# blackccpie/another_raytracer

Measured on AMD Instinct MI355X. Metric: Msamples/sec (primary+secondary rays) at 1920x1080x1024spp; 1/2/4/8 GPU, higher is better.
Workload: dtype f64

## Files before the change

another_raytracer_amd/csrc/device.h:

```cpp
#pragma once
#include <hip/hip_runtime.h>

#include <cfloat>
#include <cstdint>
#include <type_traits>

#include "glibc_log.h"
#include "layout.h"
#include "sphere_uv.h"

namespace art {

struct V3 {
    double x, y, z;
};
__device__ __forceinline__ V3 mk(double a, double b, double c) { return V3{a, b, c}; }
__device__ __forceinline__ V3 operator+(V3 u, V3 v) { return {u.x + v.x, u.y + v.y, u.z + v.z}; }
__device__ __forceinline__ V3 operator-(V3 u, V3 v) { return {u.x - v.x, u.y - v.y, u.z - v.z}; }
__device__ __forceinline__ V3 operator-(V3 u) { return {-u.x, -u.y, -u.z}; }
__device__ __forceinline__ V3 operator*(V3 u, V3 v) { return {u.x * v.x, u.y * v.y, u.z * v.z}; }
__device__ __forceinline__ V3 operator*(double t, V3 v) { return {t * v.x, t * v.y, t * v.z}; }
__device__ __forceinline__ double sqrt_rn(double x) {
    if (!(x >= 0x1p-767 && x < __builtin_inf())) return sqrt(x);
    const double y = __builtin_amdgcn_rsq(x);
    double s = x * y, h = y * 0.5;
    const double r = fma(-h, s, 0.5);
    s = fma(s, r, s);
    h = fma(h, r, h);
    s = fma(fma(-s, s, x), h, s);
    return fma(fma(-s, s, x), h, s);
}
// ... 492 lines not shown
        *(__attribute__((address_space(3))) int32_t*)(size_t)(top + kRow) = v;
        top += keep ? kRow : 0u;
    }
    __device__ __forceinline__ int32_t peek() const { return *(__attribute__((address_space(3))) const int32_t*)(size_t)top; }
    __device__ __forceinline__ void pop_if(bool c) { top -= c ? kRow : 0u; }
    __device__ __forceinline__ uint32_t save() const { return top; }
    __device__ __forceinline__ void restore(uint32_t t) { top = t; }
};
template <bool L> using StackT = typename std::conditional<L, int16_t, int32_t>::type;
template <bool L, uint32_t F> using StackF = StackT<L || (F & F_CODE16) != 0>;
template <bool L>
__device__ __forceinline__ uint32_t stack_column(uint32_t t) {
    if (!L) return t;
    return (t & ~63u) | ((t & 31u) << 1) | ((t >> 5) & 1u);
}

__device__ __forceinline__ float f32_dir(double d) {
    const float f = static_cast<float>(d);
    return __builtin_copysignf(fmaxf(__builtin_fabsf(f), 0x1p-64f), f);
}
#ifndef ART_SUSPEND_LANES
#define ART_SUSPEND_LANES 24
#endif
struct TravResume {
    int32_t node, parked;
    uint32_t sp;
    int32_t lanes;
    bool fresh;
    bool allow;
    bool suspended;
};
template <uint32_t F, int B, bool L, int PL = 0, bool RES = false, int ANY = 0>
__device__ __forceinline__ bool traverse(const DevScene& S, const uint8_t* lds, int32_t root, const Ray& r, double tmin, double tmax,
                                         StackF<L, F>* stk, double& t, uint32_t& prim, uint32_t& face, uint32_t& mt, TravResume* rs = nullptr,
                                         int32_t hoisted = kNodeEmpty) {
    static_assert(!(L && (F & F_MEDIA)), "packed LDS keys need tmin > 0: no medium boundary tests in the LDS variant");
    static_assert(!RES || !L, "resumable traversal: HBM-scene variant only");
    static_assert(ANY == 0 || !RES, "any-hit walks are never suspended");
    constexpr bool kSort = ANY != 2;
    const float ox = static_cast<float>(r.o.x), oy = static_cast<float>(r.o.y), oz = static_cast<float>(r.o.z);
    const float ix = __builtin_amdgcn_rcpf(f32_dir(r.d.x)), iy = __builtin_amdgcn_rcpf(f32_dir(r.d.y)), iz = __builtin_amdgcn_rcpf(f32_dir(r.d.z));
    const float oix = ox * ix, oiy = oy * iy, oiz = oz * iz;
    constexpr uint32_t kLdsPlane = kLdsNodeCap * 16;
    static_assert(kLdsPlane % 256 == 0, "every node plane starts on bank 0");
    const uint32_t off_nx = kLdsOffNodes + (0u + (__float_as_uint(ix) >> 31)) * kLdsPlane;
    const uint32_t off_ny = kLdsOffNodes + (3u + (__float_as_uint(iy) >> 31)) * kLdsPlane;
    const uint32_t off_nz = kLdsOffNodes + (6u + (__float_as_uint(iz) >> 31)) * kLdsPlane;
    const float tminf = f_lo(tmin);
    float tmaxf = f_hi(tmax);
    constexpr bool kSphPre = !L && (F & F_SPHERE) != 0 && (F & F_TRI) == 0;
    constexpr bool kSphLazy = kSphPre && (F & (F_BOX | F_RECT | F_XFORM | F_MEDIA)) == 0;
    const double d_a = (L || kSphPre) ? len2(r.d) : 0.0;
    double d_inv_a = (L || (kSphPre && !kSphLazy)) ? 1.0 / d_a : 0.0;
    bool hit = false;
    constexpr bool PK = !L && (F & F_CODE16) != 0;
    constexpr uint32_t kLeafShift = (PK && (F & F_LEAF2) != 0) ? 1u : 0u;
    static_assert(!PK || (F & F_MEDIA_G) == 0, "packed keys need tmin > 0: no medium boundary traversals");
    LaneStack<B, L || PK> st(stk);
    constexpr bool kNfHoist = !L && PL == 2 && ((F & F_XFORM) == 0 || (F & (F_TRI | F_MEDIA_G)) == 0);
    [[maybe_unused]] const uint32_t nf_hx = (__float_as_uint(ix) >> 31) << 4, nf_hy = (__float_as_uint(iy) >> 31) << 4,
// ... 8 lines not shown
#define ART_DPUSH(q, keep) do { if (L) { dstk[dsp] = __uint_as_float(static_cast<uint32_t>(q) & 0xFFFF0000u); dsp += (keep) ? 1 : 0; } } while (0)
#define ART_DPOP(c) do { if (L && (c)) { cur_d = dsp > 0 ? dstk[dsp - 1] : 0.0f; dsp -= dsp > 0 ? 1 : 0; } } while (0)
#else
#define ART_DPUSH(q, keep) do { } while (0)
#define ART_DPOP(c) do { } while (0)
#endif
    int32_t parked = kNodeEmpty;
    [[maybe_unused]] bool skip_nodes = false;
    if (hoisted != kNodeEmpty && (!RES || rs->fresh)) {
        const int32_t h = L ? lds_leaf(leaf_first(hoisted), leaf_count(hoisted)) : PK ? make_leaf16(leaf_first(hoisted) >> kLeafShift, leaf_count(hoisted)) : hoisted;
        parked = h;
        skip_nodes = true;
    }
    if constexpr (RES) {
        if (!rs->fresh) {
            node = rs->node;
            parked = rs->parked;
            st.restore(rs->sp);
        }
    }
    [[maybe_unused]] bool progressed = false;
    ART_STAT_LANE(6);
    for (;;) {
        if constexpr (RES) {
            if (rs->allow && progressed && __popcll(__ballot(true)) < rs->lanes) {
                rs->node = node;
                rs->parked = parked;
                rs->sp = st.save();
                rs->fresh = false;
                rs->suspended = true;
                return hit;
            }
            progressed = true;
        }
        ART_STAT_WAVE(4);
        ART_STAT_LANE(5);
        while (node >= 0 && !skip_nodes) {
            ART_STAT_WAVE(0);
            ART_STAT_LANE(1);
#ifdef ART_STATS
            if (L && cur_d > tmaxf) ART_STAT_LANE(14);
#endif
            float4 lx, hx, ly, hy, lz, hz;
            int4 ch;
            if constexpr (L) {
                const uint32_t n16 = static_cast<uint32_t>(node);
                const uint32_t ax = n16 + off_nx, ay = n16 + off_ny, az = n16 + off_nz;
// ... 441 lines not shown
                ts.h.prim = kMediumHit;
                ts.h.obj = static_cast<uint32_t>(w);
                ts.h.mt = kMatUnknown;
            }
        } else {
            uint32_t prim = 0, face = 0, mt = kMatUnknown;
            if (hit_object<F, B, false, PL, true>(S, nullptr, oi, r, 0.001, ts.closest, stk, tt, prim, face, mt, &ts.tr)) {
                ts.closest = tt;
                ts.any = true;
                ts.h.prim = prim;
                ts.h.obj = static_cast<uint32_t>(w) | (face << 16);
                ts.h.mt = mt;
            }
            if (ts.tr.suspended) {
                ts.w = w;
                return false;
            }
            ts.tr.fresh = true;
        }
    }
    return true;
}

struct Surf {
    V3 p, n;
    double u, v;
    bool ff;
    uint32_t mat;
};
__device__ __forceinline__ void set_face_normal(Surf& s, const Ray& r, V3 outward) {
    s.ff = dot(r.d, outward) < 0.0;
    s.n = s.ff ? outward : -outward;
}
__device__ __forceinline__ void face_normal(const Ray& r, V3 outward, bool& ff, V3& n) {
    ff = dot(r.d, outward) < 0.0;
    n = ff ? outward : -outward;
}
template <bool UV = true>
__device__ __forceinline__ void rect_surface(V3& p, V3& n, bool& ff, double& su, double& sv, int axis, double a0, double a1, double b0, double b1, const Ray& r,
                                             double t, bool need_uv = true) {
    if (UV && need_uv) {
        const int ia = axis == 2 ? 1 : 0;
        const int ib = axis == 0 ? 1 : 2;
        const double x = comp(r.o, ia) + t * comp(r.d, ia);
        const double y = comp(r.o, ib) + t * comp(r.d, ib);
        su = (x - a0) / (a1 - a0);
// ... 246 lines not shown
```

another_raytracer_amd/csrc/k_paths.hip:

```cpp
#include "launch.h"
#include "path_pool.h"
#include "path_work.h"
#include "tile_lists.h"

namespace art {

struct __align__(16) PoolRay {
    double2 a, b, c;
    double2 d, e;
    uint64_t rng;
    uint32_t slot, depth;
};
static_assert(sizeof(PoolRay) == 96, "pool entries are six 16-B pieces");
struct PathPool {
    PoolRay* base;
    uint32_t count;
    uint32_t cur, end;
    bool exhausted;
    __device__ __forceinline__ void init(void* pool, uint32_t block, uint32_t nblocks, uint32_t waves_per_block, uint32_t w) {
        const uint32_t per_xcd = (nblocks + kXcds - 1) / kXcds;
        const uint32_t wave = ((block % kXcds) * per_xcd + block / kXcds) * waves_per_block + w;
        base = static_cast<PoolRay*>(pool) + static_cast<size_t>(wave) * kPoolCap;
        count = cur = end = 0;
        exhausted = false;
    }
    __device__ __forceinline__ bool batch(const PassGeom& sg, const CameraRec& sc, uint32_t* next_slot, uint32_t lane, PathState& st,
                                          uint32_t& q, uint32_t& tile) {
        if (cur == end) {
            const uint32_t chunk = sg.chunk;
            uint32_t nb = 0;
            if (lane == 0) nb = atomicAdd(next_slot, chunk);
            nb = __builtin_amdgcn_readfirstlane(nb);
            cur = nb;
            end = nb + chunk;
        }
        const uint32_t b = cur;
        cur += 64;
        q = b + lane;
        __asm__ volatile("" ::: "memory");
        if (b + 64u >= sg.P) exhausted = true;
        int lx, ly;
        uint32_t qi, j;
        slot_split(sg, q, qi, j);
        tile = __builtin_amdgcn_readfirstlane(qi >> 6);
        if (!(q < sg.P && slot_pixel(sg, qi, lx, ly))) return false;
        cam_ray(sg, sc, j, lx, ly, st.ray, st.rng);
        st.T = mk(1.0, 1.0, 1.0);
        return true;
    }
    __device__ __forceinline__ void push(uint64_t m, uint32_t rank, bool busy, const PathState& st, uint32_t q, int depth) {
        if (busy) {
            PoolRay& e = base[pool_push_pos(count, rank)];
            e.a = make_double2(st.ray.o.x, st.ray.o.y);
            e.b = make_double2(st.ray.o.z, st.ray.d.x);
            e.c = make_double2(st.ray.d.y, st.ray.d.z);
            e.d = make_double2(st.ray.tm, st.T.x);
            e.e = make_double2(st.T.y, st.T.z);
            e.rng = st.rng;
            e.slot = q;
            e.depth = static_cast<uint32_t>(depth);
        }
        count += static_cast<uint32_t>(__popcll(m));
        __asm__ volatile("" ::: "memory");
    }
    __device__ __forceinline__ void pop(uint32_t rank, PathState& st, uint32_t& q, int& depth) const {
        const PoolRay& e = base[pool_pop_pos(count, rank)];
        const double2 a = e.a, b = e.b, c = e.c, d = e.d, f = e.e;
        st.ray.o = mk(a.x, a.y, b.x);
        st.ray.d = mk(b.y, c.x, c.y);
        st.ray.tm = d.x;
        st.T = mk(d.y, f.x, f.y);
        st.rng = e.rng;
        q = e.slot;
        depth = static_cast<int>(e.depth);
    }
};
typedef uint32_t u32x8 __attribute__((ext_vector_type(8)));
__device__ __forceinline__ bool trace_tile_list(const uint8_t* lds, const Ray& r, u32x8 rec, double& t, HitOut& h) {
    const double d_a = len2(r.d), d_inv_a = 1.0 / d_a;
    uint64_t q0 = rec[0] | (static_cast<uint64_t>(rec[1]) << 32), q1 = rec[2] | (static_cast<uint64_t>(rec[3]) << 32);
    uint64_t q2 = rec[4] | (static_cast<uint64_t>(rec[5]) << 32), q3 = rec[6] | (static_cast<uint64_t>(rec[7]) << 32);
    const uint32_t n = static_cast<uint32_t>(q0) & 0xFFFFu;
    double closest = __builtin_inf();
    bool any = false;
    for (uint32_t k = 0; k < n; ++k) {
        q0 = (q0 >> 16) | (q1 << 48), q1 = (q1 >> 16) | (q2 << 48), q2 = (q2 >> 16) | (q3 << 48), q3 >>= 16;
// ... 24 lines not shown
    load_lds_image<B>(S0.lds_image, smem);
    if (threadIdx.x < static_cast<uint32_t>(kJumpEntries)) jt[threadIdx.x] = pcg_jump(3u * threadIdx.x);
    if (threadIdx.x == 0) {
        s_cam = cam;
        s_g = g;
        if (g.list_mode) {
            const uint32_t n = g.list[-1];
            s_g.nlist = n;
            s_g.P = n * g.k;
        }
    }
    DevScene S = S0;
    {
        uint8_t* wb = smem + paths_lds_head(g.stack);
        uint8_t* ob = wb + sizeof(int32_t) * kPathsWorldCap;
        if (threadIdx.x < static_cast<uint32_t>(S0.nworld)) reinterpret_cast<int32_t*>(wb)[threadIdx.x] = S0.world[threadIdx.x];
        if (threadIdx.x < S0.n_objs * (sizeof(ObjRec) / 16))
            reinterpret_cast<uint4*>(ob)[threadIdx.x] = reinterpret_cast<const uint4*>(S0.objs)[threadIdx.x];
        S.world = reinterpret_cast<const int32_t*>(wb);
        S.objs = reinterpret_cast<const ObjRec*>(ob);
    }
    __syncthreads();
    const uint32_t lane = __lane_id();
    const uint64_t below = (1ull << lane) - 1ull;
    const V3 bg = mk(S.bg[0], S.bg[1], S.bg[2]);
    bool busy = false;
    uint32_t q = 0;
    int depth = 0;
    PathState st;
    unsigned long long segs = 0;
#ifdef ART_STATS
    unsigned long long tm_load = 0, tm_trace = 0, tm_shade = 0, tm_app = 0, tm_fb = 0, tm_prev = __builtin_amdgcn_s_memtime();
#endif
    const bool lists = w.tiles != nullptr && g.list == nullptr;
    uint32_t tile = 0;
    PathPool pp;
    pp.init(w.pool, blockIdx.x, gridDim.x, B / 64, threadIdx.x / 64);
    for (;;) {
        const uint64_t m_busy = __ballot(busy);
        const uint32_t n_idle = 64u - static_cast<uint32_t>(__popcll(m_busy));
        const bool fb = pool_batch_due(pp.exhausted, pp.count, n_idle);
        bool act;
        if (fb) {
#ifdef ART_STATS
            if (lane == 0) atomicAdd(&g_art_stats[51], static_cast<unsigned long long>(__popcll(m_busy)));
#endif
            if (m_busy) pp.push(m_busy, static_cast<uint32_t>(__popcll(m_busy & below)), busy, st, q, depth);
            act = pp.batch(s_g, s_cam, next_slot, lane, st, q, tile);
            depth = 0;
        } else {
            const uint32_t npop = pool_pop_count(pp.count, n_idle);
            if (npop) {
                const uint32_t rank = static_cast<uint32_t>(__popcll(~m_busy & below));
                if (!busy && rank < npop) {
                    pp.pop(rank, st, q, depth);
                    busy = true;
                }
                pp.count -= npop;
            } else if (m_busy == 0) {
                ART_TICK(tm_load);
                break;
            }
            act = busy;
        }
        ART_TICK((fb ? tm_fb : tm_load));
        double t = 0.0;
        HitOut h{0, 0, kMatUnknown};
        bool hitw = false;
        if (act) {
            ++segs;
            u32x8 rec = {kTileOverflow, 0, 0, 0, 0, 0, 0, 0};
            if (fb && lists)
                rec = *(reinterpret_cast<const __attribute__((address_space(4))) u32x8*>(reinterpret_cast<uintptr_t>(w.tiles)) +
                        __builtin_amdgcn_readfirstlane(tile));
            if ((rec[0] & 0xFFFFu) != kTileOverflow) hitw = trace_tile_list(lds, st.ray, rec, t, h);
            else hitw = trace_world<kFeatSpheres, B, true>(S, lds, st.ray, stk, st.rng, t, h);
#if ART_LDS_LEAF_NOREF
            if (hitw) h.mt = reinterpret_cast<const uint32_t*>(lds + kLdsOffRef)[h.obj >> 16] >> kLdsRefMatShift;
#endif
        }
        __asm__ volatile("s_waitcnt vmcnt(0)" ::: "memory");
        ART_TICK((fb ? tm_fb : tm_trace));
        const bool need = act && hitw && (h.mt == MAT_LAMBERTIAN || h.mt == MAT_METAL) && depth + 1 < g.max_depth;
        const V3 ps = coop_unit_sphere(need, st.rng, jt);
        bool cont = false;
        if (act) {
            st.L = mk(0.0, 0.0, 0.0);
            if (hitw) {
                cont = shade_hit_lds(lds, h.obj >> 16, h.mt, t, depth + 1 >= g.max_depth, st, &ps);
            } else {
                st.L = st.L + st.T * bg;
            }
            if (!cont) store_res(w.res, q, st.L);
        }
        ART_TICK((fb ? tm_fb : tm_shade));
#ifdef ART_STATS
        if (fb) {
            const uint64_t m_act = __ballot(act);
            if (lane == 0) {
                atomicAdd(&g_art_stats[49], 1ull);
                atomicAdd(&g_art_stats[50], static_cast<unsigned long long>(__popcll(m_act)));
            }
        }
#endif
        if (fb || act) {
            busy = cont;
            ++depth;
        }
        ART_TICK((fb ? tm_fb : tm_app));
    }
    for (int off = 32; off > 0; off >>= 1) segs += __shfl_xor(segs, off);
    if (lane == 0) atomicAdd(w.segments, segs);
#ifdef ART_STATS
    if (lane == 0) {
        atomicAdd(&g_art_stats[8], tm_load);
        atomicAdd(&g_art_stats[9], tm_trace);
        atomicAdd(&g_art_stats[10], tm_shade);
        atomicAdd(&g_art_stats[11], tm_app);
        atomicAdd(&g_art_stats[48], tm_fb);
    }
#endif
}

void launch_paths(int num_cu, hipStream_t st, const DevScene& S, const PassGeom& g, const CameraRec& cam, const Work& w,
                  uint32_t* next_slot) {
    const size_t lds = paths_lds_bytes(g.stack);
    static const bool checked = static_lds_is_zero(reinterpret_cast<const void*>(k_paths));
    (void)checked;
    (void)blocks_per_cu(reinterpret_cast<const void*>(k_paths), kBlockL, lds);
    hipLaunchKernelGGL(k_paths, dim3(num_cu), dim3(kBlockL), lds, st, S, g, cam, w, next_slot);
}
size_t pool_bytes(int variant, int num_cu) {
    return variant == EXT_MEGA ? sizeof(PoolRay) * kPoolCap * kPoolWavesPerCu * static_cast<size_t>(num_cu) : 0;
}

}
```

another_raytracer_amd/csrc/options.cpp:

```cpp
#include "options.h"

#include <algorithm>
#include <atomic>
#include <cmath>
#include <cstdlib>
#include <cstring>
#include <limits>

namespace art {

namespace {

struct OptDef {
    const char* name;
    double def, lo, hi;
    bool integer;
};
constexpr double kInf = std::numeric_limits<double>::infinity();
const OptDef kDefs[static_cast<int>(Opt::kCount)] = {
    {"compile.world_merge", 2, 0, 2, true},
    {"compile.hoist", 1, 0, 1, true},
    {"bvh.collapse", 0, 0, 1, true},
    {"bvh.collapse_ci", 0.6, 0, 1e6, false},
    {"bvh.dp_binary_leaf", 1, 1, 16, true},
    {"bvh.sah_ci", 1.5, 0, 1e6, false},
    {"bvh.sah_leaf", 4, 1, 16, true},
    {"bvh.sbvh", 1.5, 0, 1e6, false},
    {"bvh.sbvh_alpha", 1e-5, 0, 1e6, false},
    {"render.codes16", 1, 0, 1, true},
    {"render.lds_nodes_max", 4294967295.0, 0, 4294967295.0, true},
    {"render.leaf2", 1, 0, 1, true},
    {"render.tex_bary", 1, 0, 1, true},
    {"denoise.lds_iterations", 2, 0, 2, true},
    {"query.any_sorted", 0, 0, 1, true},
    {"views.max_paths", 0, 0, 2147483648.0, true},
    {"render.tile_lists", 1, 0, 2, true},
    {"render.accum_overlap", 1, 0, 2, true},
    {"grad.texel_copies", 0, 0, 64, true},
    {"multi.timeout_ms", std::numeric_limits<double>::quiet_NaN(), 0, kInf, false},
    {"multi.rccl_blocking", 0, 0, 1, true},
    {"test.fault_workspace_bytes", 0, 0, 1.8e19, true},
    {"test.fault_gather_abort", 0, 0, 1, true},
    {"test.fault_rccl_group", 0, 0, 2, true},
};

std::atomic<double> g_val[static_cast<int>(Opt::kCount)];
std::atomic<bool> g_init{false};

void init_once() {
    if (g_init.load(std::memory_order_acquire)) return;
    static const bool done = [] {
        opt_reset_all();
        g_init.store(true, std::memory_order_release);
        return true;
    }();
    (void)done;
}

int find(const char* name) {
    if (!name) return -1;
    for (int i = 0; i < static_cast<int>(Opt::kCount); ++i)
        if (std::strcmp(kDefs[i].name, name) == 0) return i;
    return -1;
}

}

void opt_reset_all() {
    for (int i = 0; i < static_cast<int>(Opt::kCount); ++i) g_val[i].store(kDefs[i].def, std::memory_order_relaxed);
}

double opt(Opt o) {
    init_once();
    const double v = g_val[static_cast<int>(o)].load(std::memory_order_relaxed);
    if (o == Opt::MultiTimeoutMs && std::isnan(v)) {
        const char* s = std::getenv("ART_MULTI_TIMEOUT_MS");
        return (!s || !*s) ? 120000.0 : std::max(0.0, std::strtod(s, nullptr));
    }
    return v;
}

bool opt_set(const char* name, double value, const char** why) {
    init_once();
    const int i = find(name);
    if (i < 0) {
        *why = "unknown option";
        return false;
    }
    const OptDef& d = kDefs[i];
    if (!(value >= d.lo && value <= d.hi) || (d.integer && value != std::floor(value))) {
        *why = d.integer ? "value outside the option's integer range" : "value outside the option's range";
        return false;
// ... 15 lines not shown
```

another_raytracer_amd/csrc/options.h:

```cpp
#pragma once
#include <cstddef>

namespace art {

enum class Opt : int {
    WorldMerge,
    Hoist,
    BvhCollapse,
    CollapseCi,
    DpBinaryLeaf,
    SahCi,
    SahLeaf,
    Sbvh,
    SbvhAlpha,
    Codes16,
    LdsNodesMax,
    Leaf2,
    TexBary,
    DenoiseLdsIterations,
    QueryAnySorted,
    ViewsMaxPaths,
    TileLists,
    AccumOverlap,
    GradTexelCopies,
    MultiTimeoutMs,
    RcclBlocking,
    FaultWorkspaceBytes,
    FaultGatherAbort,
    FaultRcclGroup,
    kCount
};

double opt(Opt o);
bool opt_set(const char* name, double value, const char** why);
bool opt_get(const char* name, double* value);
void opt_reset_all();

}
```

another_raytracer_amd/csrc/path_work.h:

```cpp
#pragma once
#include <hip/hip_runtime.h>

#include <cstdint>

#include "device.h"
#include "pass_plan.h"

namespace art {

struct PathRec {
    double2 a, b, c, e;
    double2 f, g, h, i;
};
static_assert(sizeof(PathRec) == 128, "PathRec is two 64-B lines");
struct PathState {
    Ray ray;
    V3 T, L;
    uint64_t rng;
};
__device__ __forceinline__ void load_path(const PathRec* P, uint32_t q, PathState& s, bool full) {
    const PathRec& p = P[q];
    const double2 a = p.a, b = p.b, c = p.c, e = p.e;
    s.ray.o = mk(a.x, a.y, b.x);
    s.ray.d = mk(b.y, c.x, c.y);
    s.ray.tm = e.x;
// ... 50 lines not shown

struct FastDiv {
    uint32_t d, m, l;
    static FastDiv make(uint32_t d) {
        uint32_t l = 0;
        while (l < 32 && (1ull << l) < d) ++l;
        return FastDiv{d, static_cast<uint32_t>(((1ull << 32) * ((1ull << l) - d)) / d + 1), l};
    }
    __device__ __forceinline__ uint32_t div(uint32_t n) const { return (__umulhi(m, n) + n) >> l; }
};

struct PassGeom {
    int32_t W, H;
    int32_t rows;
    int32_t band_rows, band_count, band_index;
    uint32_t tiles_x, npix_pad;
    uint32_t k;
    uint32_t sample_base;
    uint32_t P;
    uint32_t cap;
    uint32_t live;
    uint32_t stack;
    int32_t max_depth;
    uint64_t seed;
    uint64_t seed_mix;
    FastDiv fd_npix, fd_tiles_x, fd_band_rows, fd_w;
    double inv_w1, inv_h1;
    const uint32_t* list;
    uint32_t nlist;
    uint32_t chunk;
    uint32_t lds_ring;
    uint32_t list_mode;
};
struct Work {
    PathRec* paths;
    HitRecD* hits;
    ResRec* res;
    uint32_t* active[2];
    uint32_t* mq;
    uint32_t* counters;
    unsigned long long* segments;
    double* acc;
    void* pool;
    const void* tiles;
};
__host__ __device__ __forceinline__ uint32_t* counter(const Work& w, int d, int kind, int s) {
    return w.counters + (static_cast<size_t>((d * kQueueKinds + kind) * kShards + s)) * kCounterStride;
}

__device__ __forceinline__ int global_row(const PassGeom& g, int ly) {
    const uint32_t b = g.fd_band_rows.div(static_cast<uint32_t>(ly));
    return static_cast<int>(b) * (g.band_rows * g.band_count) + g.band_index * g.band_rows + (ly - static_cast<int>(b) * g.band_rows);
}
__device__ __forceinline__ void slot_split(const PassGeom& g, uint32_t slot, uint32_t& qi, uint32_t& j) {
    const uint32_t a = g.fd_npix.div(slot), b = slot - a * g.npix_pad;
    qi = g.list_mode ? a : b;
// ... 271 lines not shown
```

another_raytracer_amd/csrc/renderer.hip:

```cpp
#include "renderer.h"

#include <algorithm>
#include <cstdio>
#include <cstdlib>
#include <cstring>
#include <vector>

#include "call_plan.h"
#include "launch.h"
#include "lds_image.h"
#include "options.h"
#include "pass_plan.h"
#include "refit.h"
#include "tile_lists.h"
#include "view_plan.h"
#include "workspace.h"

namespace art {

struct Renderer::Impl {
    int device = 0;
    int num_cu = 256;
    hipStream_t own_stream = nullptr;
    FlatScene flat;
// ... 118 lines not shown
        unsigned long long segments = 0;
        void fill(RenderStats* s, uint64_t primary, int passes, int samples_per_pass) const {
            if (s) *s = RenderStats{}, s->segments = segments, s->primary = primary, s->ms = ms, s->passes = passes, s->samples_per_pass = samples_per_pass;
        }
    };
    Done finish(const unsigned long long* d_segments = nullptr) {
        Done d;
        if (timed && d_segments) HIP_OK(hipMemcpyAsync(&d.segments, d_segments, sizeof d.segments, hipMemcpyDeviceToHost, st));
        if (wait) HIP_OK(hipStreamSynchronize(st));
        if (timed) HIP_OK(hipEventElapsedTime(&d.ms, ev[0], ev[1]));
        return d;
    }
};
static uint64_t slot_target(const Renderer::Impl& I, size_t slot_bytes) {
    size_t free_b = 0, total_b = 0;
    HIP_OK(hipMemGetInfo(&free_b, &total_b));
    return slot_target(free_b, I.ws.size(), slot_bytes);
}

size_t Renderer::scene_bytes() const { return impl_->s64.bytes; }
int Renderer::device() const { return impl_->device; }
const FlatScene& Renderer::flat() const { return impl_->flat; }

static PassGeom make_pass_geom(const RenderParams& p, int nrows, uint32_t stack) {
    PassGeom g{};
    g.W = p.width;
    g.H = p.height;
    g.rows = nrows;
    g.band_rows = p.band_rows;
    g.band_count = p.band_count;
    g.band_index = p.band_index;
    g.tiles_x = static_cast<uint32_t>((p.width + 7) / 8);
    const uint32_t tiles_y = static_cast<uint32_t>((nrows + 7) / 8);
    g.npix_pad = g.tiles_x * tiles_y * 64u;
    g.max_depth = p.max_depth;
    g.seed = p.seed;
    g.seed_mix = splitmix64(p.seed);
    g.fd_tiles_x = FastDiv::make(g.tiles_x);
    g.fd_band_rows = FastDiv::make(static_cast<uint32_t>(p.band_rows));
    g.fd_w = FastDiv::make(static_cast<uint32_t>(p.width));
    g.fd_npix = FastDiv::make(g.npix_pad);
    g.inv_w1 = 1.0 / static_cast<double>(p.width - 1);
    g.inv_h1 = 1.0 / static_cast<double>(p.height - 1);
    g.stack = stack;
    return g;
}
constexpr uint32_t kTileListsAutoSpp = 72;
static bool tile_lists_wanted(const DeviceScene& ds, int variant, uint32_t k) {
    const int mode = static_cast<int>(opt(Opt::TileLists));
    return variant == EXT_MEGA && ds.tile_reps > 0 && (mode == 2 || (mode == 1 && k >= kTileListsAutoSpp));
}
static size_t counter_words(int max_depth) { return static_cast<size_t>(std::max(max_depth + 1, 4)) * kQueueKinds * kShards * kCounterStride; }

struct ProfileMarks {
    std::vector<hipEvent_t> ev;
    size_t used = 0;
    ~ProfileMarks() { for (auto e : ev) if (e) (void)hipEventDestroy(e); }
    void reserve(size_t n) {
        while (ev.size() < n) {
            ev.push_back(nullptr);
            HIP_OK(hipEventCreate(&ev.back()));
        }
    }
    void mark(hipStream_t stream) {
        reserve(used + 1);
        HIP_OK(hipEventRecord(ev[used++], stream));
    }
// ... 82 lines not shown
    f.stream = f.call.st;
    for (int a = 0; a < 3; ++a) f.ds.view.bg[a] = p.background[a];
    f.nrows = band_local_rows(p.height, p.band_rows, p.band_count, p.band_index);
    stats.local_rows = f.nrows;
    if (f.nrows == 0) return false;
    f.g = make_pass_geom(p, f.nrows, stack_rows(f.ds.max_stack));
    f.variant = extend_variant(f.ds, p.flags);
    f.mega = f.variant == EXT_MEGA || f.variant == EXT_MEGA_G;
    const size_t slot_bytes = f.mega ? sizeof(ResRec) : sizeof(PathRec) + sizeof(HitRecD) + sizeof(ResRec) + 4u * (2u + kNumMatTypes) + 8u;
    const uint64_t target = slot_target(I, slot_bytes);
    if (f.g.npix_pad > kMaxPassSlots) throw std::runtime_error("image too large for one pass (more than 2^31 padded pixels)");
    const PassPlan plan = plan_passes(target, p.samples_per_pass, f.g.npix_pad, spp, spread);
    f.k = plan.k, f.npasses = plan.npasses;
    f.Pmax = f.k * f.g.npix_pad;
    f.g.cap = shard_cap(f.Pmax);
    f.local_pix = static_cast<size_t>(f.nrows) * p.width;
    f.counter_bytes = f.mega ? 4u * kCounterStride : 4ull * counter_words(p.max_depth);
    f.call.carve(I.ws, carve);
    if (p.flags & RT_PROFILE) {
        f.marks.reserve(static_cast<size_t>(profile_levels) * f.npasses * (f.variant == EXT_MEGA ? 4 : f.mega ? 2 : 3 * p.max_depth));
        f.mark = [&f]() { f.marks.mark(f.stream); };
    }
    f.call.begin();
    HIP_OK(hipMemsetAsync(f.w.segments, 0, sizeof(unsigned long long), f.stream));
    if (p.max_depth == 0) HIP_OK(hipMemsetAsync(f.w.res, 0, sizeof(ResRec) * f.Pmax, f.stream));
    return true;
}

static void run_pass(Frame& f, PassGeom g, int line = 0, bool clear = true, size_t res_first = 0) {
    Work w = f.w;
    w.res += res_first;
    if (clear) HIP_OK(hipMemsetAsync(f.w.counters, 0, f.counter_bytes, f.stream));
    if (!f.mega) {
        for (int d = 0; d < f.p.max_depth; ++d) bounce(f.ds, f.variant, f.I.num_cu, f.stream, g, f.cam, w, d, f.mark);
        f.launches += static_cast<uint64_t>(f.p.max_depth);
    } else if (f.p.max_depth > 0) {
        g.chunk = path_chunk(g.P, f.I.num_cu);
        if (f.mark) f.mark();
        if (f.variant == EXT_MEGA) {
            launch_paths(f.I.num_cu, f.stream, f.ds.view, g, f.cam, w, counter(w, line, 0, 0));
            f.kid = KernelId{kFeatSpheres, 0, 3};
        } else {
            f.kid = launch_paths_g(f.ds.features, f.ds.tex_basic, f.ds.tex_bary, f.ds.codes16, f.ds.leaf_shift, f.I.num_cu, f.stream, f.ds.view, g,
                                   f.cam, w, counter(w, line, 0, 0));
        }
        if (f.mark) f.mark();
        ++f.launches;
    }
    ++f.passes;
}

static PassGeom list_geom(PassGeom g, const uint32_t* list, uint32_t nlist, uint32_t k, uint32_t sample_base, uint32_t P) {
    g.list_mode = 1, g.list = list, g.nlist = nlist;
    g.k = g.npix_pad = k, g.fd_npix = FastDiv::make(k), g.sample_base = sample_base;
    g.P = g.live = P;
    return g;
}

static void end_frame(Frame& f, RenderStats& stats, uint8_t* out_rgb, double* out_acc, const std::function<void()>& more_copies = {}) {
#ifdef ART_STATS
    HIP_OK(hipGetLastError());
    dump_art_stats(f.stream);
#endif
    f.call.end();
    f.call.copy_out(out_rgb, f.drgb, 3 * f.local_pix);
    f.call.copy_out(out_acc, f.w.acc, sizeof(double) * 3 * f.local_pix);
    if (more_copies) more_copies();
    const Call::Done done = f.call.finish(f.w.segments);
    stats.ms = done.ms, stats.segments = done.segments, stats.passes = f.passes, stats.samples_per_pass = static_cast<int>(f.k);
    stats.extend_variant = f.variant, stats.kernel_features = f.kid.f, stats.kernel_textures = f.kid.tf, stats.kernel_lds_mode = f.kid.lm;
    if (f.p.flags & RT_PROFILE) {
        f.marks.sum(f.mega ? 2 : 3, stats.extend_ms, stats.shade_ms);
        stats.extend_launches = f.launches;
        stats.shade_launches = f.variant == EXT_GLOBAL || f.variant == EXT_LDS ? f.launches : 0;
    }
}

struct RenderBufs {
    int spp_t;
    uint8_t* out_rgb;
    double *out_acc, *qsum;
    int32_t* ad_work;
    uint32_t *ad_lists, *ad_count;
    uint8_t *ad_f0, *ad_f1, *ad_f2;
    int sqx;
    uint32_t nsq;
};

static int trace_samples(Frame& f, const RenderBufs& b, const uint32_t* list, uint32_t nlist) {
    const RenderParams& p = f.p;
    PassGeom g = f.g;
// ... 102 lines not shown
}

void Renderer::render(const CameraRec& cam, const RenderParams& p, uint8_t* out_rgb, double* out_acc, RenderStats& stats) {
    if (p.fp_mode != RT_FP64) throw std::runtime_error("fp_mode must be RT_FP64");
    upload();
    Impl& I = *impl_;
    Frame f{I, I.s64, cam, p};
    const bool images = (p.flags & RT_PARALLEL_IMAGES) != 0, adaptive = (p.flags & RT_ADAPTIVE) != 0;
    RenderBufs b{};
    b.spp_t = images ? 4 * (p.spp / 4) : p.spp, b.out_rgb = out_rgb, b.out_acc = out_acc;
#ifdef ART_TRACE
    trace_setup();
#endif
    TileRec* tile_tab = nullptr;
    if (!begin_frame(f, stats, b.spp_t, true, adaptive ? 4 : 1, [&](Carver& c) {
        const bool wf = !f.mega;
        f.w.paths = c.take<PathRec>(f.Pmax, wf);
        f.w.hits = c.take<HitRecD>(f.Pmax, wf);
        f.w.res = c.take<ResRec>(f.Pmax);
        f.w.active[0] = c.take<uint32_t>(static_cast<size_t>(kShards) * f.g.cap, wf);
        f.w.active[1] = c.take<uint32_t>(static_cast<size_t>(kShards) * f.g.cap, wf);
        f.w.mq = c.take<uint32_t>(static_cast<size_t>(kMatSegs) * f.g.cap, wf);
        f.w.counters = c.take<uint32_t>(counter_words(p.max_depth));
        f.w.segments = c.take<unsigned long long>(1);
        f.w.acc = c.take<double>(3 * f.local_pix);
        f.drgb = c.take<uint8_t>(3 * f.local_pix);
        double* qsum = c.take<double>(3 * f.local_pix, images);
        b.qsum = images ? qsum : nullptr;
        f.w.pool = c.take<char>(pool_bytes(f.variant, I.num_cu));
        tile_tab = c.take<TileRec>(f.g.npix_pad / 64u, !adaptive && tile_lists_wanted(f.ds, f.variant, f.k));
        b.ad_work = c.take<int32_t>(3 * f.local_pix, adaptive);
        b.ad_lists = c.take<uint32_t>(adaptive_list_words(static_cast<uint32_t>(f.local_pix / (kBig * kBig))), adaptive);
        b.ad_f0 = c.take<uint8_t>(21 * (f.local_pix / (kBig * kBig)), adaptive);
        b.ad_count = c.take<uint32_t>(1, adaptive);
    })) return;
    b.ad_f1 = b.ad_f0 + f.local_pix / (kBig * kBig), b.ad_f2 = b.ad_f1 + 4 * (f.local_pix / (kBig * kBig));
    b.sqx = p.width / kBig, b.nsq = static_cast<uint32_t>(b.sqx) * static_cast<uint32_t>(f.nrows / kBig);
    uint32_t ad_counts[4] = {0, 0, 0, 0};
    uint64_t primary = 0;
    if (!adaptive && p.max_depth > 0 && tile_lists_wanted(f.ds, f.variant, f.k)) {
        launch_tile_lists(f.stream, f.ds.view, f.g, cam, tile_tab);
        f.w.tiles = tile_tab;
    }
    if (!adaptive) primary = render_whole(f, b);
    else if (f.mega && f.k == static_cast<uint32_t>(b.spp_t) && !images && !p.on_pass) adaptive_device_counted(f, b, ad_counts);
    else primary = adaptive_host_counted(f, b);
    end_frame(f, stats, out_rgb, adaptive ? nullptr : out_acc);
// ... 279 lines not shown
    DeviceBuffer tmp;
    double* d_rays = nullptr;
    uint64_t* d_rng = nullptr;
    call.carve(tmp, [&](Carver& c) { d_rays = call.out(c, rays_out, 7 * ne), d_rng = call.out(c, rng_out, ne); }, 1);
    launch_camera_rays(call.st, g, cam, d_rays, d_rng);
    call.end();
    call.finish();
}

void Renderer::render_noise_target(const CameraRec& cam, const RenderParams& p, const NoiseParams& np, uint8_t* out_rgb, double* out_acc,
                                   int32_t* out_count, double* out_moments, RenderStats& stats, NoiseResult& result) {
    if (p.fp_mode != RT_FP64) throw std::runtime_error("fp_mode must be RT_FP64");
    upload();
    Impl& I = *impl_;
    Frame f{I, I.s64, cam, p};
    result = NoiseResult{};
    double* mom = nullptr;
    int32_t* count = nullptr;
    uint8_t* flag = nullptr;
    uint32_t *list_base = nullptr, *conv = nullptr;
    if (!begin_frame(f, stats, p.spp, false, 0, [&](Carver& c) {
        f.w.res = c.take<ResRec>(f.Pmax);
        f.w.counters = c.take<uint32_t>(kCounterStride);
        f.w.segments = c.take<unsigned long long>(1);
        f.w.acc = c.take<double>(3 * f.local_pix);
        mom = c.take<double>(2 * f.local_pix);
        count = c.take<int32_t>(f.local_pix);
        flag = c.take<uint8_t>(f.local_pix);
        f.drgb = c.take<uint8_t>(3 * f.local_pix);
        list_base = c.take<uint32_t>(nt_list_words(f.local_pix));
        conv = c.take<uint32_t>(1);
        f.w.pool = c.take<char>(pool_bytes(f.variant, I.num_cu));
    })) return;
    if (!f.mega) throw std::runtime_error("internal: noise-target rendering needs a persistent-path kernel");
    hipStream_t stream = f.stream;
    const Work& w = f.w;
    const size_t local_pix = f.local_pix;
    const uint32_t npix = static_cast<uint32_t>(local_pix), tile_pad = f.g.npix_pad;
    const double* res = reinterpret_cast<const double*>(w.res);
    uint32_t* lists[2] = {list_base + 64, list_base + nt_list_stride(local_pix) + 64};
    HIP_OK(hipMemsetAsync(w.acc, 0, sizeof(double) * 3 * local_pix, stream));
    HIP_OK(hipMemsetAsync(mom, 0, sizeof(double) * 2 * local_pix, stream));
    HIP_OK(hipMemsetAsync(flag, 0, local_pix, stream));
    HIP_OK(hipMemsetAsync(list_base, 0, 4 * nt_list_words(local_pix), stream));
    HIP_OK(hipMemsetAsync(conv, 0, 4, stream));
    const uint32_t min_spp = static_cast<uint32_t>(np.min_spp), cap_spp = static_cast<uint32_t>(p.spp), step = static_cast<uint32_t>(np.step_spp);
    PassGeom g = f.g;
// ... 281 lines not shown
```

Baseline: 23820.

## Suspend partial LDS BVH walks into the path pool when wave occupancy drops

Lets the persistent-path kernel's LDS-scene traversal suspend when fewer than a threshold of lanes are active. The partial walk (closest t, node, parked leaf, world index, short stack) is saved into a new per-wave PoolWalk area beside the pooled rays, so idle lanes can be refilled with fresh paths and suspended walks are resumed later. The aim is to cut SIMD divergence from long-tail traversals. In exchange it adds pool memory, per-iteration ballots, stack copy traffic and new bookkeeping for which pool slots hold walks. The hold threshold defaults to 8 lanes through a new option, and diagnostic counters for held and displaced paths are added.

```diff
diff --git a/another_raytracer_amd/csrc/device.h b/another_raytracer_amd/csrc/device.h
--- a/another_raytracer_amd/csrc/device.h
+++ b/another_raytracer_amd/csrc/device.h
@@ -7,6 +7,7 @@
 
 #include "glibc_log.h"
 #include "layout.h"
+#include "path_hold.h"
 #include "sphere_uv.h"
 
 namespace art {
@@ -545,6 +546,8 @@
 #ifndef ART_SUSPEND_LANES
 #define ART_SUSPEND_LANES 24
 #endif
+template <int B>
+__host__ __device__ constexpr uint32_t hold_stack_row(uint32_t depth) { return kLdsImageBytes + depth * 2u * B; }
 struct TravResume {
     int32_t node, parked;
     uint32_t sp;
@@ -558,7 +561,6 @@
                                          StackF<L, F>* stk, double& t, uint32_t& prim, uint32_t& face, uint32_t& mt, TravResume* rs = nullptr,
                                          int32_t hoisted = kNodeEmpty) {
     static_assert(!(L && (F & F_MEDIA)), "packed LDS keys need tmin > 0: no medium boundary tests in the LDS variant");
-    static_assert(!RES || !L, "resumable traversal: HBM-scene variant only");
     static_assert(ANY == 0 || !RES, "any-hit walks are never suspended");
     constexpr bool kSort = ANY != 2;
     const float ox = static_cast<float>(r.o.x), oy = static_cast<float>(r.o.y), oz = static_cast<float>(r.o.z);
@@ -613,7 +615,19 @@
     [[maybe_unused]] bool progressed = false;
     ART_STAT_LANE(6);
     for (;;) {
-        if constexpr (RES) {
+        if constexpr (RES && L) {
+            const bool more = (node != kNodeEmpty || parked != kNodeEmpty) &&
+                              static_cast<int32_t>(st.top) < static_cast<int32_t>(hold_stack_row<B>(kHoldStackCap + 1));
+            if (rs->allow && progressed && __popcll(__ballot(true)) < rs->lanes && more) {
+                rs->node = node;
+                rs->parked = parked;
+                rs->sp = st.save();
+                rs->fresh = false;
+                rs->suspended = true;
+                return hit;
+            }
+            progressed = true;
+        } else if constexpr (RES) {
             if (rs->allow && progressed && __popcll(__ballot(true)) < rs->lanes) {
                 rs->node = node;
                 rs->parked = parked;
@@ -1101,6 +1115,29 @@
     return true;
 }
 
+template <uint32_t F, int B>
+__device__ __forceinline__ bool trace_world_res_lds(const DevScene& S, const uint8_t* lds, const Ray& r, StackT<true>* stk, TraceState& ts) {
+    ts.tr.suspended = false;
+    for (int32_t w = ts.w; w < S.nworld; ++w) {
+        const int32_t oi = S.world[w];
+        double tt;
+        uint32_t prim = 0, face = 0, mt = kMatUnknown;
+        if (hit_object<F, B, true, 0, true>(S, lds, oi, r, 0.001, ts.closest, stk, tt, prim, face, mt, &ts.tr)) {
+            ts.closest = tt;
+            ts.any = true;
+            ts.h.prim = prim;
+            ts.h.obj = static_cast<uint32_t>(w) | (face << 16);
+            ts.h.mt = mt;
+        }
+        if (ts.tr.suspended) {
+            ts.w = w;
+            return false;
+        }
+        ts.tr.fresh = true;
+    }
+    return true;
+}
+
 struct Surf {
     V3 p, n;
     double u, v;
diff --git a/another_raytracer_amd/csrc/k_paths.hip b/another_raytracer_amd/csrc/k_paths.hip
--- a/another_raytracer_amd/csrc/k_paths.hip
+++ b/another_raytracer_amd/csrc/k_paths.hip
@@ -12,18 +12,34 @@
     uint32_t slot, depth;
 };
 static_assert(sizeof(PoolRay) == 96, "pool entries are six 16-B pieces");
+struct __align__(16) PoolWalk {
+    double t;
+    uint32_t np;
+    uint32_t misc;
+    uint32_t stk[kHoldStackCap / 2];
+};
+static_assert(sizeof(PoolWalk) == 64, "walk entries are four 16-B pieces");
+static_assert(kPathsWorldCap <= kWalkWorldCap, "walk_pack's world slots (path_hold.h)");
+constexpr unsigned long long kSegsDisplaced = 1ull << 40;
+constexpr size_t kPoolWaveBytes = (sizeof(PoolRay) + sizeof(PoolWalk)) * kPoolCap;
+__device__ __forceinline__ uint32_t lanes_below(uint64_t m) {
+    return __builtin_amdgcn_mbcnt_hi(static_cast<uint32_t>(m >> 32), __builtin_amdgcn_mbcnt_lo(static_cast<uint32_t>(m), 0u));
+}
 struct PathPool {
     PoolRay* base;
+    uint64_t held;
     uint32_t count;
     uint32_t cur, end;
     bool exhausted;
     __device__ __forceinline__ void init(void* pool, uint32_t block, uint32_t nblocks, uint32_t waves_per_block, uint32_t w) {
         const uint32_t per_xcd = (nblocks + kXcds - 1) / kXcds;
-        const uint32_t wave = ((block % kXcds) * per_xcd + block / kXcds) * waves_per_block + w;
-        base = static_cast<PoolRay*>(pool) + static_cast<size_t>(wave) * kPoolCap;
+        const uint32_t wave = ((block % kXcds) * per_xcd + block / kXcds) * waves_per_block + __builtin_amdgcn_readfirstlane(w);
+        base = reinterpret_cast<PoolRay*>(static_cast<uint8_t*>(pool) + static_cast<size_t>(wave) * kPoolWaveBytes);
+        held = 0;
         count = cur = end = 0;
         exhausted = false;
     }
+    __device__ __forceinline__ PoolWalk* walks() const { return reinterpret_cast<PoolWalk*>(base + kPoolCap); }
     __device__ __forceinline__ bool batch(const PassGeom& sg, const CameraRec& sc, uint32_t* next_slot, uint32_t lane, PathState& st,
                                           uint32_t& q, uint32_t& tile) {
         if (cur == end) {
@@ -48,7 +64,31 @@
         st.T = mk(1.0, 1.0, 1.0);
         return true;
     }
-    __device__ __forceinline__ void push(uint64_t m, uint32_t rank, bool busy, const PathState& st, uint32_t q, int depth) {
+    __device__ __forceinline__ void push(uint64_t m, uint64_t m_held, bool busy, bool walk, const PathState& st, uint32_t q,
+                                         int depth, double t, uint32_t np, uint32_t misc, const StackT<true>* stk) {
+        const uint32_t n_held = static_cast<uint32_t>(__popcll(m_held));
+        const uint32_t rank = hold_push_rank(walk, lanes_below(m_held), n_held, lanes_below(m & ~m_held));
+        if (m_held) {
+            if (walk) {
+                PoolWalk& x = walks()[pool_push_pos(count, rank)];
+                *reinterpret_cast<uint4*>(&x) = make_uint4(static_cast<uint32_t>(__double_as_longlong(t)),
+                                                           static_cast<uint32_t>(__double_as_longlong(t) >> 32), np, misc);
+                const uint32_t n = walk_entries(misc);
+                for (uint32_t k0 = 0; k0 < kHoldStackCap; k0 += 8) {
+                    if (k0 >= n) break;
+                    uint32_t v[4];
+#pragma unroll
+                    for (uint32_t c = 0; c < 4; ++c) {
+                        const uint32_t k = k0 + 2 * c;
+                        const uint32_t lo = k < n ? static_cast<uint16_t>(stk[k * kBlockL]) : 0u;
+                        const uint32_t hi = k + 1 < n ? static_cast<uint16_t>(stk[(k + 1) * kBlockL]) : 0u;
+                        v[c] = lo | (hi << 16);
+                    }
+                    *reinterpret_cast<uint4*>(&x.stk[k0 / 2]) = make_uint4(v[0], v[1], v[2], v[3]);
+                }
+            }
+            held = hold_mask_push(held, count, n_held);
+        }
         if (busy) {
             PoolRay& e = base[pool_push_pos(count, rank)];
             e.a = make_double2(st.ray.o.x, st.ray.o.y);
@@ -62,6 +102,25 @@
         }
         count += static_cast<uint32_t>(__popcll(m));
         __asm__ volatile("" ::: "memory");
+    }
+    __device__ __forceinline__ void pop_walk(uint32_t pos, double& t, uint32_t& np, uint32_t& misc, StackT<true>* stk) const {
+        const PoolWalk& x = walks()[pos];
+        const uint4 hd = *reinterpret_cast<const uint4*>(&x);
+        t = __longlong_as_double(static_cast<long long>(hd.x | (static_cast<uint64_t>(hd.y) << 32)));
+        np = hd.z;
+        misc = hd.w;
+        const uint32_t n = walk_entries(misc);
+        for (uint32_t k0 = 0; k0 < kHoldStackCap; k0 += 8) {
+            if (k0 >= n) break;
+            const uint4 s = *reinterpret_cast<const uint4*>(&x.stk[k0 / 2]);
+            const uint32_t v[4] = {s.x, s.y, s.z, s.w};
+#pragma unroll
+            for (uint32_t c = 0; c < 4; ++c) {
+                const uint32_t k = k0 + 2 * c;
+                if (k < n) stk[k * kBlockL] = static_cast<StackT<true>>(v[c] & 0xFFFFu);
+                if (k + 1 < n) stk[(k + 1) * kBlockL] = static_cast<StackT<true>>(v[c] >> 16);
+            }
+        }
     }
     __device__ __forceinline__ void pop(uint32_t rank, PathState& st, uint32_t& q, int& depth) const {
         const PoolRay& e = base[pool_pop_pos(count, rank)];
@@ -132,13 +191,18 @@
     }
     __syncthreads();
     const uint32_t lane = __lane_id();
-    const uint64_t below = (1ull << lane) - 1ull;
     const V3 bg = mk(S.bg[0], S.bg[1], S.bg[2]);
     bool busy = false;
     uint32_t q = 0;
     int depth = 0;
     PathState st;
     unsigned long long segs = 0;
+    bool walk = false;
+    uint32_t w_np = 0, w_misc = 0;
+    double t = 0.0;
+    const uint32_t col2 = 2u * stack_column<true>(threadIdx.x);
+    constexpr uint32_t kRow = LaneStack<B, true>::kRow;
+    const int32_t hold_lanes = static_cast<int32_t>(g.hold + (g.hold >= 64u ? 1u : 0u));
 #ifdef ART_STATS
     unsigned long long tm_load = 0, tm_trace = 0, tm_shade = 0, tm_app = 0, tm_fb = 0, tm_prev = __builtin_amdgcn_s_memtime();
 #endif
@@ -155,18 +219,32 @@
 #ifdef ART_STATS
             if (lane == 0) atomicAdd(&g_art_stats[51], static_cast<unsigned long long>(__popcll(m_busy)));
 #endif
-            if (m_busy) pp.push(m_busy, static_cast<uint32_t>(__popcll(m_busy & below)), busy, st, q, depth);
+            if (m_busy) {
+                const uint64_t m_walk = __ballot(walk);
+                segs += static_cast<unsigned long long>(__popcll(m_walk)) * kSegsDisplaced;
+                pp.push(m_busy, m_walk, busy, walk, st, q, depth, t, w_np, w_misc, stk);
+            }
             act = pp.batch(s_g, s_cam, next_slot, lane, st, q, tile);
             depth = 0;
+            walk = false;
         } else {
             const uint32_t npop = pool_pop_count(pp.count, n_idle);
             if (npop) {
-                const uint32_t rank = static_cast<uint32_t>(__popcll(~m_busy & below));
-                if (!busy && rank < npop) {
+                const uint32_t rank = lanes_below(~m_busy);
+                const bool take = !busy && rank < npop;
+                const uint32_t pos = pool_pop_pos(pp.count, rank);
+                if (take) {
                     pp.pop(rank, st, q, depth);
                     busy = true;
                 }
                 pp.count -= npop;
+                if (hold_mask_popped(pp.held, pp.count)) {
+                    if (take && hold_mask_has(pp.held, pos)) {
+                        pp.pop_walk(pos, t, w_np, w_misc, stk);
+                        walk = true;
+                    }
+                    pp.held = hold_mask_keep(pp.held, pp.count);
+                }
             } else if (m_busy == 0) {
                 ART_TICK(tm_load);
                 break;
@@ -174,27 +252,59 @@
             act = busy;
         }
         ART_TICK((fb ? tm_fb : tm_load));
-        double t = 0.0;
+        const bool allow = !fb && !(pp.exhausted && pp.count == 0);
         HitOut h{0, 0, kMatUnknown};
         bool hitw = false;
+#define WALK_NONE(...) __asm__ volatile("" : __VA_ARGS__)
+        const bool resume = walk && act;
+        walk = false;
+        if (!act) WALK_NONE("=v"(w_np), "=v"(w_misc), "=v"(t));
+        segs += static_cast<unsigned long long>(__popcll(__ballot(act && !resume)));
         if (act) {
-            ++segs;
             u32x8 rec = {kTileOverflow, 0, 0, 0, 0, 0, 0, 0};
             if (fb && lists)
                 rec = *(reinterpret_cast<const __attribute__((address_space(4))) u32x8*>(reinterpret_cast<uintptr_t>(w.tiles)) +
                         __builtin_amdgcn_readfirstlane(tile));
-            if ((rec[0] & 0xFFFFu) != kTileOverflow) hitw = trace_tile_list(lds, st.ray, rec, t, h);
-            else hitw = trace_world<kFeatSpheres, B, true>(S, lds, st.ray, stk, st.rng, t, h);
-#if ART_LDS_LEAF_NOREF
+            if ((rec[0] & 0xFFFFu) != kTileOverflow) {
+                hitw = trace_tile_list(lds, st.ray, rec, t, h);
+                WALK_NONE("=v"(w_np), "=v"(w_misc));
+            } else {
+                TraceState ts;
+                ts.start();
+                ts.h = h;
+                if (resume) {
+                    ts.closest = t;
+                    ts.any = walk_any(w_misc);
+                    ts.h.obj = walk_obj(w_misc);
+                    ts.w = walk_world(w_misc);
+                    ts.tr.node = walk_node(w_np);
+                    ts.tr.parked = walk_parked(w_np);
+                    ts.tr.sp = hold_stack_row<B>(0) + col2 + (walk_depth1(w_misc) - 1u) * kRow;
+                    ts.tr.fresh = false;
+                }
+                ts.tr.allow = allow;
+                ts.tr.lanes = hold_lanes;
+                walk = !trace_world_res_lds<kFeatSpheres, B>(S, lds, st.ray, stk, ts);
+                hitw = ts.any;
+                t = ts.closest;
+                h = ts.h;
+                if (walk) {
+                    w_np = walk_pack_np(ts.tr.node, ts.tr.parked);
+                    w_misc = walk_pack(h.obj, ts.w, (ts.tr.sp - hold_stack_row<B>(0) + kRow) / kRow, hitw);
+                } else {
+                    WALK_NONE("=v"(w_np), "=v"(w_misc));
+                }
+            }
             if (hitw) h.mt = reinterpret_cast<const uint32_t*>(lds + kLdsOffRef)[h.obj >> 16] >> kLdsRefMatShift;
-#endif
-        }
+        }
+#undef WALK_NONE
         __asm__ volatile("s_waitcnt vmcnt(0)" ::: "memory");
         ART_TICK((fb ? tm_fb : tm_trace));
-        const bool need = act && hitw && (h.mt == MAT_LAMBERTIAN || h.mt == MAT_METAL) && depth + 1 < g.max_depth;
+        const bool sh = act && !walk;
+        const bool need = sh && hitw && (h.mt == MAT_LAMBERTIAN || h.mt == MAT_METAL) && depth + 1 < g.max_depth;
         const V3 ps = coop_unit_sphere(need, st.rng, jt);
         bool cont = false;
-        if (act) {
+        if (sh) {
             st.L = mk(0.0, 0.0, 0.0);
             if (hitw) {
                 cont = shade_hit_lds(lds, h.obj >> 16, h.mt, t, depth + 1 >= g.max_depth, st, &ps);
@@ -213,14 +323,16 @@
             }
         }
 #endif
-        if (fb || act) {
+        if (fb || sh) {
             busy = cont;
             ++depth;
         }
         ART_TICK((fb ? tm_fb : tm_app));
     }
-    for (int off = 32; off > 0; off >>= 1) segs += __shfl_xor(segs, off);
-    if (lane == 0) atomicAdd(w.segments, segs);
+    if (lane == 0) {
+        atomicAdd(w.segments, segs & (kSegsDisplaced - 1ull));
+        if (segs >= kSegsDisplaced) atomicAdd(w.segments + 1, segs / kSegsDisplaced);
+    }
 #ifdef ART_STATS
     if (lane == 0) {
         atomicAdd(&g_art_stats[8], tm_load);
@@ -241,7 +353,7 @@
     hipLaunchKernelGGL(k_paths, dim3(num_cu), dim3(kBlockL), lds, st, S, g, cam, w, next_slot);
 }
 size_t pool_bytes(int variant, int num_cu) {
-    return variant == EXT_MEGA ? sizeof(PoolRay) * kPoolCap * kPoolWavesPerCu * static_cast<size_t>(num_cu) : 0;
-}
-
-}
+    return variant == EXT_MEGA ? kPoolWaveBytes * kPoolWavesPerCu * static_cast<size_t>(num_cu) : 0;
+}
+
+}
diff --git a/another_raytracer_amd/csrc/options.cpp b/another_raytracer_amd/csrc/options.cpp
--- a/another_raytracer_amd/csrc/options.cpp
+++ b/another_raytracer_amd/csrc/options.cpp
@@ -36,12 +36,15 @@
     {"views.max_paths", 0, 0, 2147483648.0, true},
     {"render.tile_lists", 1, 0, 2, true},
     {"render.accum_overlap", 1, 0, 2, true},
+    {"render.paths_hold", 8, 0, 64, true},
     {"grad.texel_copies", 0, 0, 64, true},
     {"multi.timeout_ms", std::numeric_limits<double>::quiet_NaN(), 0, kInf, false},
     {"multi.rccl_blocking", 0, 0, 1, true},
     {"test.fault_workspace_bytes", 0, 0, 1.8e19, true},
     {"test.fault_gather_abort", 0, 0, 1, true},
     {"test.fault_rccl_group", 0, 0, 2, true},
+    {"diag.paths_held", 0, 0, 1.8e19, true},
+    {"diag.paths_displaced", 0, 0, 1.8e19, true},
 };
 
 std::atomic<double> g_val[static_cast<int>(Opt::kCount)];
@@ -68,6 +71,12 @@
 
 void opt_reset_all() {
     for (int i = 0; i < static_cast<int>(Opt::kCount); ++i) g_val[i].store(kDefs[i].def, std::memory_order_relaxed);
+}
+
+void opt_note_paths_held(unsigned long long held, unsigned long long displaced) {
+    init_once();
+    g_val[static_cast<int>(Opt::DiagPathsHeld)].store(static_cast<double>(held), std::memory_order_relaxed);
+    g_val[static_cast<int>(Opt::DiagPathsDisplaced)].store(static_cast<double>(displaced), std::memory_order_relaxed);
 }
 
 double opt(Opt o) {
diff --git a/another_raytracer_amd/csrc/options.h b/another_raytracer_amd/csrc/options.h
--- a/another_raytracer_amd/csrc/options.h
+++ b/another_raytracer_amd/csrc/options.h
@@ -22,12 +22,15 @@
     ViewsMaxPaths,
     TileLists,
     AccumOverlap,
+    PathsHold,
     GradTexelCopies,
     MultiTimeoutMs,
     RcclBlocking,
     FaultWorkspaceBytes,
     FaultGatherAbort,
     FaultRcclGroup,
+    DiagPathsHeld,
+    DiagPathsDisplaced,
     kCount
 };
 
@@ -35,5 +38,6 @@
 bool opt_set(const char* name, double value, const char** why);
 bool opt_get(const char* name, double* value);
 void opt_reset_all();
+void opt_note_paths_held(unsigned long long held, unsigned long long displaced);
 
 }
diff --git a/another_raytracer_amd/csrc/path_hold.h b/another_raytracer_amd/csrc/path_hold.h
--- /dev/null
+++ b/another_raytracer_amd/csrc/path_hold.h
@@ -0,0 +1,36 @@
+#pragma once
+#include <cstdint>
+
+#include "layout.h"
+
+namespace art {
+
+constexpr uint32_t kHoldStackCap = 24;
+static_assert(kHoldStackCap % 8 == 0, "the stack travels in 16-B pieces of eight entries");
+
+constexpr uint32_t kWalkObjMask = 0xFFFF000Fu;
+constexpr uint32_t kWalkWorldCap = 16;
+static_assert(kHoldStackCap + 2 < 128, "walk_pack's depth field");
+ART_HD uint32_t walk_pack_np(int32_t node, int32_t parked) {
+    return (static_cast<uint32_t>(node) & 0xFFFFu) | (static_cast<uint32_t>(parked) << 16);
+}
+ART_HD int32_t walk_node(uint32_t np) { return static_cast<int16_t>(np & 0xFFFFu); }
+ART_HD int32_t walk_parked(uint32_t np) { return static_cast<int32_t>(np) >> 16; }
+ART_HD uint32_t walk_pack(uint32_t obj, int32_t w, uint32_t depth1, bool any) {
+    return (obj & kWalkObjMask) | (static_cast<uint32_t>(w) << 4) | (depth1 << 8) | (any ? 0x8000u : 0u);
+}
+ART_HD uint32_t walk_obj(uint32_t misc) { return misc & kWalkObjMask; }
+ART_HD int32_t walk_world(uint32_t misc) { return static_cast<int32_t>((misc >> 4) & 15u); }
+ART_HD uint32_t walk_depth1(uint32_t misc) { return (misc >> 8) & 127u; }
+ART_HD bool walk_any(uint32_t misc) { return (misc & 0x8000u) != 0; }
+ART_HD uint32_t walk_entries(uint32_t misc) { return walk_depth1(misc) > 1u ? walk_depth1(misc) - 1u : 0u; }
+
+ART_HD uint32_t hold_push_rank(bool walk, uint32_t walk_below, uint32_t n_walk, uint32_t other_below) {
+    return walk ? walk_below : n_walk + other_below;
+}
+ART_HD uint64_t hold_mask_push(uint64_t mask, uint32_t count, uint32_t n_walk) { return mask | (((1ull << n_walk) - 1ull) << count); }
+ART_HD bool hold_mask_popped(uint64_t mask, uint32_t count) { return (mask >> count) != 0; }
+ART_HD uint64_t hold_mask_keep(uint64_t mask, uint32_t count) { return mask & ((1ull << count) - 1ull); }
+ART_HD bool hold_mask_has(uint64_t mask, uint32_t pos) { return ((mask >> pos) & 1ull) != 0; }
+
+}
diff --git a/another_raytracer_amd/csrc/path_work.h b/another_raytracer_amd/csrc/path_work.h
--- a/another_raytracer_amd/csrc/path_work.h
+++ b/another_raytracer_amd/csrc/path_work.h
@@ -1,6 +1,7 @@
 #pragma once
 #include <hip/hip_runtime.h>
 
+#include <cstddef>
 #include <cstdint>
 
 #include "device.h"
@@ -97,6 +98,7 @@
     uint32_t live;
     uint32_t stack;
     int32_t max_depth;
+    uint32_t hold;
     uint64_t seed;
     uint64_t seed_mix;
     FastDiv fd_npix, fd_tiles_x, fd_band_rows, fd_w;
@@ -107,6 +109,7 @@
     uint32_t lds_ring;
     uint32_t list_mode;
 };
+static_assert(sizeof(PassGeom) == 168 && offsetof(PassGeom, seed) == 64, "PassGeom::hold took the padding: the kernels' argument layout is unchanged");
 struct Work {
     PathRec* paths;
     HitRecD* hits;
diff --git a/another_raytracer_amd/csrc/renderer.hip b/another_raytracer_amd/csrc/renderer.hip
--- a/another_raytracer_amd/csrc/renderer.hip
+++ b/another_raytracer_amd/csrc/renderer.hip
@@ -164,6 +164,7 @@
 int Renderer::device() const { return impl_->device; }
 const FlatScene& Renderer::flat() const { return impl_->flat; }
 
+constexpr size_t kSegmentWords = 3;
 static PassGeom make_pass_geom(const RenderParams& p, int nrows, uint32_t stack) {
     PassGeom g{};
     g.W = p.width;
@@ -185,6 +186,7 @@
     g.inv_w1 = 1.0 / static_cast<double>(p.width - 1);
     g.inv_h1 = 1.0 / static_cast<double>(p.height - 1);
     g.stack = stack;
+    g.hold = static_cast<uint32_t>(opt(Opt::PathsHold));
     return g;
 }
 constexpr uint32_t kTileListsAutoSpp = 72;
@@ -313,7 +315,7 @@
         f.mark = [&f]() { f.marks.mark(f.stream); };
     }
     f.call.begin();
-    HIP_OK(hipMemsetAsync(f.w.segments, 0, sizeof(unsigned long long), f.stream));
+    HIP_OK(hipMemsetAsync(f.w.segments, 0, kSegmentWords * sizeof(unsigned long long), f.stream));
     if (p.max_depth == 0) HIP_OK(hipMemsetAsync(f.w.res, 0, sizeof(ResRec) * f.Pmax, f.stream));
     return true;
 }
@@ -357,7 +359,10 @@
     f.call.copy_out(out_rgb, f.drgb, 3 * f.local_pix);
     f.call.copy_out(out_acc, f.w.acc, sizeof(double) * 3 * f.local_pix);
     if (more_copies) more_copies();
+    unsigned long long held[2] = {0, 0};
+    if (f.call.timed && f.variant == EXT_MEGA) HIP_OK(hipMemcpyAsync(held, f.w.segments + 1, sizeof held, hipMemcpyDeviceToHost, f.stream));
     const Call::Done done = f.call.finish(f.w.segments);
+    if (f.call.timed && f.call.wait && f.variant == EXT_MEGA) opt_note_paths_held(held[0], held[1]);
     stats.ms = done.ms, stats.segments = done.segments, stats.passes = f.passes, stats.samples_per_pass = static_cast<int>(f.k);
     stats.extend_variant = f.variant, stats.kernel_features = f.kid.f, stats.kernel_textures = f.kid.tf, stats.kernel_lds_mode = f.kid.lm;
     if (f.p.flags & RT_PROFILE) {
@@ -506,7 +511,7 @@
         f.w.active[1] = c.take<uint32_t>(static_cast<size_t>(kShards) * f.g.cap, wf);
         f.w.mq = c.take<uint32_t>(static_cast<size_t>(kMatSegs) * f.g.cap, wf);
         f.w.counters = c.take<uint32_t>(counter_words(p.max_depth));
-        f.w.segments = c.take<unsigned long long>(1);
+        f.w.segments = c.take<unsigned long long>(kSegmentWords);
         f.w.acc = c.take<double>(3 * f.local_pix);
         f.drgb = c.take<uint8_t>(3 * f.local_pix);
         double* qsum = c.take<double>(3 * f.local_pix, images);
@@ -832,7 +837,7 @@
     if (!begin_frame(f, stats, p.spp, false, 0, [&](Carver& c) {
         f.w.res = c.take<ResRec>(f.Pmax);
         f.w.counters = c.take<uint32_t>(kCounterStride);
-        f.w.segments = c.take<unsigned long long>(1);
+        f.w.segments = c.take<unsigned long long>(kSegmentWords);
         f.w.acc = c.take<double>(3 * f.local_pix);
         mom = c.take<double>(2 * f.local_pix);
         count = c.take<int32_t>(f.local_pix);
```

Result: slower. 22740 (-4.6%).
